# mehta-lab/dynamorph

Measured on AMD Instinct MI355X. Metric: cell-patches/sec (128x128x2) VQ-VAE fwd+bwd, higher is better.
Workload: dtype f32; 1 GPU; C3: VQ_VAE training step (forward + backward + fused Adam), 2x128x128 fp32 synthetic patches; per_gpu_batch=2048, global_batch=2048, parallelism=dp1, hip_graph=True, fused_trainer=True, backward_products=f32

## Files before the change

### dynamorph_amd/csrc/conv_mfma.hip

```cpp
#include "dm_common.h"
#include "tile.h"
#include "mfma_util.h"

int dm_generic_conv_slabs(int B, int per_tile);
int dm_generic_conv(int form, const Operand &in, const WeightView &wv, float *out, const Epilogue &ep, int B, int Cphys,
                    int CIN, int NOUT, int H, int W, int taps, int nslabs, int per_tile, hipStream_t st);
bool dm_wide_conv_ok(int form, int H, int W);
int dm_wide_conv_slabs(int form, int B, int H, int W, int per_tile);
long long dm_wide_conv_scratch_floats(int form, int CIN, int NOUT, int taps);
int dm_wide_conv(int form, const Operand &in, const WeightView &wv, float *scratch, float *out, const Epilogue &ep, int B,
                 int Cphys, int CIN, int NOUT, int H, int W, int taps, int nslabs, int per_tile, hipStream_t st);

bool dm_conv4x4s2_patch_forward(const Operand &in, const WeightView &wv, float *out, const Epilogue &ep, int B, int Cphys, int CIN,
                                int NOUT, int H, int W, int per_tile, int nslabs, hipStream_t stream, int *rc);

namespace {

enum { SIDE_NONE = 0, SIDE_MASK = 1, SIDE_ALL = 2 };

template <int SIDE> struct EpiIn { f32x4 m; };
template <> struct EpiIn<SIDE_ALL> { f32x4 m, r, q; };

constexpr unsigned DM_RSRC_FLAGS = 0x00020000u;
constexpr int DM_VOFF_NONE = 0x40000000;
// ... 533 lines not shown
        }
    }
    if (ep.stats && !(NPASS == 1 && per_tile)) {
        stats_reduce<NTT, PIX>(s1, s2, s_stat, ep, CO, blockIdx.x);
        zero_unowned_slabs(ep, CO, nslabs);
    }
}

template <int CIN, int COUT, int TH, int TW, bool TWO, int SIDE, int WPS>
__global__ __launch_bounds__(DM_BLOCK, WPS)
void convT_phase_kernel(Operand in, WeightView wv, float *__restrict__ out, Epilogue ep, int Cphys, int H, int W,
                        int ntiles, int nslabs)
{
    static_assert(COUT == 8 || COUT == 16, "built for 8 or 16 output channels");
    constexpr int IH = TH + 2, RS = TW + 8, COLS4 = RS / 4;
    constexpr int PSRAW = IH * RS;
    constexpr int PS = PSRAW + ((16 - (PSRAW % 32)) + 32) % 32;
    constexpr int CG = TW / 16, MT = TH * CG, MTW = MT / 4, MP = 2;
    constexpr int NPX = COUT == 16 ? 2 : 1;
    constexpr int TAPX = COUT == 16 ? 2 : 3;
    constexpr int KS = (CIN / 4) * 2 * TAPX;
    static_assert(CIN % 4 == 0 && MTW % MP == 0 && MTW >= MP, "shape");
    __shared__ __attribute__((aligned(16))) float tile[CIN * PS];
    __shared__ __attribute__((aligned(16))) float s_coef[DM_COEF_MAX_C * 4];
    __shared__ double s_stat[4 * 16][2];

    const int tiles_x = W / TW, tiles_y = H / TH;
    const int lane = threadIdx.x & 63, wave = threadIdx.x >> 6, m = lane & 15, kq = lane >> 4;
    const int OH = 2 * H, OW = 2 * W;
    const int co = COUT == 16 ? m : (m & 7), pxl = COUT == 16 ? 0 : (m >> 3);

    TileStage<CIN, IH, COLS4, RS, PS, TWO> stage;
    stage.init(H, W);
    int tidx = blockIdx.x, b = 0, y0 = 0, x0 = 0;
    if (tidx < ntiles) {
        int t = tidx;
        x0 = (t % tiles_x) * TW; t /= tiles_x;
        y0 = (t % tiles_y) * TH; b = t / tiles_y;
        stage.issue(in, b, Cphys, H, W, y0 - 1, x0 - 4);
        stage_coef(s_coef, in, b, Cphys);
    }

    float wreg[2][NPX][1][KS];
#pragma unroll
    for (int py = 0; py < 2; ++py)
#pragma unroll
        for (int pxt = 0; pxt < NPX; ++pxt)
#pragma unroll
            for (int s = 0; s < KS; ++s) {
                const int cg4 = s / (2 * TAPX), j = s % (2 * TAPX), a = j / TAPX, bb = j % TAPX;
                const int c = 4 * cg4 + kq;
                const int px = COUT == 16 ? pxt : pxl;
                const int row = py + a, col = COUT == 16 ? pxt + bb : bb;
                const int ky = py + 3 - 2 * row, kx = px + 3 - 2 * col;
                float wvl = 0.f;
                if (ky >= 0 && ky <= 3 && kx >= 0 && kx <= 3) wvl = wv.w[wv.off + co * wv.sn + c * wv.sc + ky * wv.sky + kx * wv.skx];
                wreg[py][pxt][0][s] = wvl;
            }
    const float bias = ep.bias ? ep.bias[co] : 0.f;
    float mc0, mc2;
    mask_coef(ep, 0, co, mc0, mc2);

    double s1 = 0.0, s2 = 0.0;
    const int abase = kq * PS + m + 3;
    EpiCtx<SIDE> cx;
    const long long sample_elems = (long long)COUT * OH * OW;
    const int chan_off = (co * OH * OW + 8 * kq + 4 * pxl) * 4;

    while (tidx < ntiles) {
        __syncthreads();
        stage.commit(tile, s_coef, Cphys, H, W, y0 - 1, x0 - 4, in.mode);
        __syncthreads();
        const int cb = b, cy0 = y0, cx0 = x0;
        const int next = tidx + gridDim.x;
        {
            int t = next < ntiles ? next : tidx;
            x0 = (t % tiles_x) * TW; t /= tiles_x;
            y0 = (t % tiles_y) * TH; b = t / tiles_y;
        }
        const auto scx = stage.begin(in, next < ntiles, b, Cphys, H, W, y0 - 1, x0 - 4);
        const bool recoef = next < ntiles && coef_changes(in, cb, b);
        f32x4 cfn = {1.f, 0.f, 0.f, 0.f};
        if (recoef) cfn = coef_fetch(in, b, Cphys);
        if (SIDE != SIDE_NONE && ep.mask.p0 && ep.mask.coef_bstride) mask_coef(ep, cb, co, mc0, mc2);
        cx.rebase(ep, out, sample_elems, cb);
        constexpr int NP = MTW / MP, NE = decltype(stage)::N;
#pragma unroll
        for (int p = 0; p < NP; ++p) {
#pragma unroll
            for (int e = 0; e < NE; ++e)
                if (e >= p * NE / NP && e < (p + 1) * NE / NP) stage.issue_one(e, scx);
            const float *ap[MP];
            int obase[MP];
#pragma unroll
            for (int i = 0; i < MP; ++i) {
                const int ti = wave + 4 * (MP * p + i);
                const int r = ti / CG, cg = ti % CG;
                ap[i] = tile + r * RS + 16 * cg + abase;
                obase[i] = chan_off + (2 * (cy0 + r) * OW + 2 * (cx0 + 16 * cg)) * 4;
            }
#pragma unroll
            for (int py = 0; py < 2; ++py) {
                EpiIn<SIDE> e[MP][NPX];
#pragma unroll
                for (int i = 0; i < MP; ++i)
#pragma unroll
                    for (int h = 0; h < NPX; ++h) epilogue_loads<SIDE>(e[i][h], cx, obase[i] + py * OW * 4 + 16 * h);
                f32x4 acc[NPX][MP][1];
#pragma unroll
                for (int pxt = 0; pxt < NPX; ++pxt) {
#pragma unroll
                    for (int i = 0; i < MP; ++i) acc[pxt][i][0] = (f32x4){0.f, 0.f, 0.f, 0.f};
                    auto off = [py, pxt](int s) {
                        const int cg4 = s / (2 * TAPX), j = s % (2 * TAPX), a = j / TAPX, bb = j % TAPX;
                        return 4 * cg4 * PS + (py + a) * RS + (COUT == 16 ? pxt + bb : bb);
                    };
                    mfma_tiles<MP, 1, KS, TAPX * 2>(ap, wreg[py][pxt], acc[pxt], off);
                }
#pragma unroll
                for (int i = 0; i < MP; ++i) {
                    if constexpr (COUT == 16) {
                        const f32x4 v0 = bias_relu(acc[0][i][0], ep, bias), v1 = bias_relu(acc[1][i][0], ep, bias);
                        epilogue_tail<SIDE>((f32x4){v0.x, v1.x, v0.y, v1.y}, ep, cx, e[i][0], mc0, mc2,
                                            obase[i] + py * OW * 4, s1, s2);
                        epilogue_tail<SIDE>((f32x4){v0.z, v1.z, v0.w, v1.w}, ep, cx, e[i][1], mc0, mc2,
                                            obase[i] + py * OW * 4 + 16, s1, s2);
                    } else {
                        const f32x4 v = bias_relu(acc[0][i][0], ep, bias);
                        const f32x4 pv = lane_xor8(v);
                        epilogue_tail<SIDE>(pxl ? (f32x4){pv.z, v.z, pv.w, v.w} : (f32x4){v.x, pv.x, v.y, pv.y}, ep, cx,
                                            e[i][0], mc0, mc2, obase[i] + py * OW * 4, s1, s2);
                    }
                }
            }
        }
        if (recoef) coef_put(s_coef, in, cfn, Cphys);
        tidx = next;
    }
    if (ep.stats) {
        double a = s1, c = s2;
        a += __shfl_xor(a, 16, 64); c += __shfl_xor(c, 16, 64);
        a += __shfl_xor(a, 32, 64); c += __shfl_xor(c, 32, 64);
        if (COUT == 8) { a += __shfl_xor(a, 8, 64); c += __shfl_xor(c, 8, 64); }
        if (lane < COUT) { s_stat[wave * 16 + lane][0] = a; s_stat[wave * 16 + lane][1] = c; }
        __syncthreads();
        if (threadIdx.x < COUT) {
            double ta = 0.0, tc = 0.0;
#pragma unroll
            for (int w = 0; w < 4; ++w) { ta += s_stat[w * 16 + threadIdx.x][0]; tc += s_stat[w * 16 + threadIdx.x][1]; }
            ep.stats[((long long)blockIdx.x * COUT + threadIdx.x) * 2 + 0] = ta;
            ep.stats[((long long)blockIdx.x * COUT + threadIdx.x) * 2 + 1] = tc;
        }
        zero_unowned_slabs(ep, COUT, nslabs);
    }
}

template <int CD, int CX, int TH, int TW>
struct FusedBwdGeom {
    static_assert(CD == 16 && CX == 8 && (TH == 8 || TH == 4) && TW % 16 == 0, "built for enc.4: 8 -> 16 channels");
    static constexpr int IH = TH + 2, RS = TW + 8, COLS4 = RS / 4, PSRAW = IH * RS;
    static constexpr int PS = PSRAW + ((16 - (PSRAW % 32)) + 32) % 32;
    static constexpr int TROWS = 2 * TH + 2, RST = 2 * TW + 8, TCOLS4 = RST / 4, PST = TROWS * RST;
    static constexpr int N = CX * 16, NTT = N / 16;
    static constexpr int TILE_FLOATS = CD * PS + CX * PST, RED_FLOATS = NTT * 256;
    static constexpr size_t LDS_BYTES = (size_t)(2 * TILE_FLOATS + 2 * DM_COEF_MAX_C * 4) * 4 + 8 * 16 * 2 * sizeof(double);
    static_assert(RED_FLOATS <= TILE_FLOATS, "the slab combine reuses a tile buffer");
};

template <int CD, int CX, int TH, int TW, bool ZF, bool DESC>
__global__ __launch_bounds__(768, 1)
void bwd_s2_roles3_kernel(Operand dy, Operand tin, WeightView wv, float *__restrict__ dx, Epilogue ep,
                         float *__restrict__ wslabs, int H, int W, int ntiles, int dbg)
{
    using G = FusedBwdGeom<CD, CX, TH, TW>;
    constexpr int RW = 4;
    constexpr int IH = G::IH, RS = G::RS, COLS4 = G::COLS4, PS = G::PS;
    constexpr int TROWS = G::TROWS, RST = G::RST, TCOLS4 = G::TCOLS4, PST = G::PST, NTT = G::NTT, N = G::N;
    constexpr int BUF = CD * PS + CX * PST;
    constexpr int CGN = TW / 16, MP = ZF ? CGN : 2, NPASS = TH * CGN / (RW * MP), WROWS = TH / RW;
    static_assert(TH * CGN == RW * MP * NPASS && TH == RW * WROWS, "tile split over the waves of a role");
    constexpr int TAPX = 3, KS = (CD / 4) * 2 * TAPX;
    extern __shared__ __attribute__((aligned(16))) float fb_lds[];
    float *s_coefD = fb_lds + 2 * BUF, *s_coefT = s_coefD + DM_COEF_MAX_C * 4;
    double (*s_stat)[2] = reinterpret_cast<double (*)[2]>(s_coefT + DM_COEF_MAX_C * 4);

    const int lane = threadIdx.x & 63, m = lane & 15, kq = lane >> 4;
    const int wave = __builtin_amdgcn_readfirstlane(threadIdx.x >> 6);
    const int role = wave / RW;
    const int rw = wave & (RW - 1);
    const int OH = 2 * H, OW = 2 * W;
    const int tiles_x = W / TW, tiles_y = H / TH;
    auto coords = [&](int kth, int &tb, int &ty0, int &tx0) {
        int t = tile_id<DESC>(kth, ntiles);
        tx0 = (t % tiles_x) * TW; t /= tiles_x;
        ty0 = (t % tiles_y) * TH; tb = t / tiles_y;
    };
    stage_coef(s_coefD, dy, 0, CD);
    stage_coef(s_coefT, tin, 0, CX);
    int tidx = blockIdx.x;

    if (role == 1) {
        TileStage<CD, IH, COLS4, RS, PS, true, 256> stD;
        TileStage<CX, TROWS, TCOLS4, RST, PST, false, 256> stT;
        const int tl = (int)threadIdx.x - 256;
        stD.init(H, W, tl);
        stT.init(OH, OW, tl);
        int b, y0, x0;
        if (tidx < ntiles) {
            coords(tidx, b, y0, x0);
            stD.issue(dy, b, CD, H, W, y0 - 1, x0 - 4);
        }
        __syncthreads();
        if (tidx < ntiles) {
            stD.commit(fb_lds, s_coefD, CD, H, W, y0 - 1, x0 - 4, dy.mode);
            stT.issue(tin, b, CX, OH, OW, 2 * y0 - 1, 2 * x0 - 4);
            stT.commit(fb_lds + CD * PS, s_coefT, CX, OH, OW, 2 * y0 - 1, 2 * x0 - 4, tin.mode);
        }
        __syncthreads();
        int p = 0;
        while (tidx < ntiles) {
            const int next = tidx + gridDim.x;
            float *nxt = fb_lds + (1 - p) * BUF;
            int nb = 0, ny0 = 0, nx0 = 0;
            if (next < ntiles && !(dbg & 4)) {
                coords(next, nb, ny0, nx0);
                stD.issue(dy, nb, CD, H, W, ny0 - 1, nx0 - 4);
                stD.commit(nxt, s_coefD, CD, H, W, ny0 - 1, nx0 - 4, dy.mode);
                stT.issue(tin, nb, CX, OH, OW, 2 * ny0 - 1, 2 * nx0 - 4);
                stT.commit(nxt + CD * PS, s_coefT, CX, OH, OW, 2 * ny0 - 1, 2 * nx0 - 4, tin.mode);
            }
            __syncthreads();
            p ^= 1;
            tidx = next;
        }
        for (int w = 0; w < RW + 2; ++w) __syncthreads();
    } else if (role == 2) {
        int bl[NTT];
#pragma unroll
        for (int t = 0; t < NTT; ++t) {
            const int n = 16 * t + m;
            bl[t] = CD * PS + (n >> 4) * PST + ((n >> 2) & 3) * RST + (n & 3) + 3 + 8 * kq + 2 * rw * RST;
        }
        const int al = m * PS + (rw + 1) * RS + 4 + 4 * kq;
        f32x4 wacc[NTT];
#pragma unroll
        for (int t = 0; t < NTT; ++t) wacc[t] = (f32x4){0.f, 0.f, 0.f, 0.f};
        __syncthreads();
        __syncthreads();
        int p = 0;
        while (tidx < ntiles) {
            const float *cur = fb_lds + p * BUF;
            if (!(dbg & 1)) {
                constexpr int NSPAN = TW / 16, NQ = WROWS * NSPAN * 4;
                auto aoff = [](int q) { return (q / (NSPAN * 4)) * RW * RS + 16 * ((q >> 2) % NSPAN); };
                auto boff = [](int q) { return (q / (NSPAN * 4)) * RW * 2 * RST + 32 * ((q >> 2) % NSPAN) + 2 * (q & 3); };
                f32x4 av[2];
                float bv[2][NTT];
                av[0] = *reinterpret_cast<const f32x4 *>(cur + al);
#pragma unroll
                for (int t = 0; t < NTT; ++t) bv[0][t] = cur[bl[t]];
#pragma unroll
                for (int q = 0; q < NQ; ++q) {
                    if (q + 1 < NQ) {
                        if (((q + 1) & 3) == 0) av[((q + 1) >> 2) & 1] = *reinterpret_cast<const f32x4 *>(cur + al + aoff(q + 1));
#pragma unroll
                        for (int t = 0; t < NTT; ++t) bv[(q + 1) & 1][t] = cur[bl[t] + boff(q + 1)];
                    }
                    __builtin_amdgcn_sched_barrier(0);
                    const float a = av[(q >> 2) & 1][q & 3];
#pragma unroll
                    for (int t = 0; t < NTT; ++t) wacc[t] = __builtin_amdgcn_mfma_f32_16x16x4f32(a, bv[q & 1][t], wacc[t], 0, 0, 0);
                    __builtin_amdgcn_sched_barrier(0);
                }
            }
            __syncthreads();
            p ^= 1;
            tidx += gridDim.x;
        }
        float *red = fb_lds;
        for (int w = 0; w < RW; ++w) {
            __syncthreads();
            if (rw == w) {
#pragma unroll
                for (int t = 0; t < NTT; ++t) {
                    f32x4 *pp = reinterpret_cast<f32x4 *>(red + (t * 64 + lane) * 4);
                    if (w == 0) *pp = wacc[t];
                    else *pp = *pp + wacc[t];
                }
            }
        }
        __syncthreads();
        __syncthreads();
    } else {
        const int co = m & 7, pxl = m >> 3;
        constexpr int NTW = ZF ? 2 : 1, KSW = ZF ? (CD / 4) * 2 : KS;
        float wreg[2][NTW][KSW];
#pragma unroll
        for (int py = 0; py < 2; ++py)
#pragma unroll
            for (int t = 0; t < NTW; ++t)
#pragma unroll
                for (int s = 0; s < KSW; ++s) {
                    int cg4, a, kx;
                    if constexpr (ZF) { cg4 = s >> 1; a = s & 1; kx = t == 0 ? 1 + pxl : (pxl ? 0 : 3); }
                    else { cg4 = s / (2 * TAPX); const int j = s % (2 * TAPX); a = j / TAPX; kx = pxl + 3 - 2 * (j % TAPX); }
                    const int c = 4 * cg4 + kq;
// ... 82 lines not shown
            p ^= 1;
            tidx += gridDim.x;
        }
        for (int w = 0; w < RW + 1; ++w) __syncthreads();
        if (ep.stats) {
            double a = s1, c = s2;
            a += __shfl_xor(a, 16, 64); c += __shfl_xor(c, 16, 64);
            a += __shfl_xor(a, 32, 64); c += __shfl_xor(c, 32, 64);
            a += __shfl_xor(a, 8, 64); c += __shfl_xor(c, 8, 64);
            if (lane < CX) { s_stat[rw * 16 + lane][0] = a; s_stat[rw * 16 + lane][1] = c; }
        }
        __syncthreads();
        if (ep.stats && threadIdx.x < CX) {
            double ta = 0.0, tc = 0.0;
#pragma unroll
            for (int w = 0; w < RW; ++w) { ta += s_stat[w * 16 + threadIdx.x][0]; tc += s_stat[w * 16 + threadIdx.x][1]; }
            ep.stats[((long long)blockIdx.x * CX + threadIdx.x) * 2 + 0] = ta;
            ep.stats[((long long)blockIdx.x * CX + threadIdx.x) * 2 + 1] = tc;
        }
    }
    float *slab = wslabs + (long long)blockIdx.x * (CD * N);
    for (int i = threadIdx.x; i < NTT * 256; i += 768) {
        const int j = i & 3, l = (i >> 2) & 63, t = i >> 8;
        slab[(4 * (l >> 4) + j) * N + 16 * t + (l & 15)] = fb_lds[i];
    }
}

struct ConvArgs {
    Operand in; WeightView wv; float *out; Epilogue ep;
    int B, Cphys, CIN, NOUT, H, W, per_tile;
    int ntiles, nslabs;
    hipStream_t stream;
};

int side_mode(const Epilogue &ep)
{
    if (!ep.mask.p0 && !ep.resid && !ep.stat_q) return SIDE_NONE;
    if (ep.mask.p0 && !ep.resid && (!ep.stat_q || ep.stat_q == ep.mask.p0)) return SIDE_MASK;
    return SIDE_ALL;
}

int conv_grid(int ntiles, int wgs_per_cu, int per_tile, int npass = 1)
{
    if (per_tile && npass > 1) return ntiles;
    const int cap = 256 * wgs_per_cu;
    return ntiles < cap ? ntiles : cap;
}

int conv_slabs(int ntiles, int per_tile) { return per_tile ? ntiles : (ntiles < 256 * 3 ? ntiles : 256 * 3); }

constexpr int lds_wgs(int lds_bytes) { return (160 * 1024) / (lds_bytes + 3072); }
constexpr int clampi(int v, int lo, int hi) { return v < lo ? lo : (v > hi ? hi : v); }

constexpr int conv_wps(int lds_bytes, int weights, int tile_f4, bool two, int mp, int nt, int side)
{
    const int stage = ((tile_f4 + DM_BLOCK - 1) / DM_BLOCK) * (two ? 9 : 5);
    const int epi = mp * nt * (6 + (side == SIDE_ALL ? 12 : (side == SIDE_MASK ? 4 : 0)));
    const int est = weights + stage + epi + 48;
    return clampi(lds_wgs(lds_bytes), 1, est > 145 ? 2 : 3);
}

int conv4_tw(int CIN, int Wo)
{
    const int cap = CIN <= 5 ? 64 : (CIN <= 8 ? 32 : 16);
    return Wo < cap ? Wo : cap;
}

constexpr bool CONV4_DESC = true;
constexpr bool FUSED_BWD_DESC = true;

template <int CIN, int TW>
void launch_conv4(const ConvArgs &a)
{
    constexpr int TH = 8;
    constexpr int F4 = CIN * (2 * TH + 2) * ((2 * TW + 8) / 4), LDS = 16 * F4;
#define DM_L4(SIDE_)                                                                                              \
    {                                                                                                             \
        constexpr int WPS = conv_wps(LDS, CIN * 4, F4, false, 2, 1, SIDE_);                                       \
                                            \
        if (SIDE_ == SIDE_NONE && CIN <= 4 && TW == 64 && a.NOUT == 8 && a.ep.bias_border && !a.ep.relu)          \
            hipLaunchKernelGGL((conv4x4s2_pair_kernel<CIN <= 4 ? CIN : 1, TH, WPS>),                              \
                               dim3(conv_grid(a.ntiles, WPS, a.per_tile)), dim3(DM_BLOCK), 0, a.stream, a.in, a.wv, \
                               a.out, a.ep, a.Cphys, a.H, a.W, a.ntiles, a.nslabs, a.per_tile);                   \
        else if (SIDE_ == SIDE_NONE && CIN <= 5 && a.ep.bias_border)                                              \
            hipLaunchKernelGGL((conv4x4s2_kernel<CIN, 1, TH, TW, SIDE_NONE, WPS, true, CONV4_DESC>),              \
                               dim3(conv_grid(a.ntiles, WPS, a.per_tile)), dim3(DM_BLOCK), 0, a.stream, a.in, a.wv, \
                               a.out, a.ep, a.Cphys, a.NOUT, a.H, a.W, a.ntiles, a.nslabs,                        \
                               a.per_tile);                                                                       \
        else                                                                                                      \
            hipLaunchKernelGGL((conv4x4s2_kernel<CIN, 1, TH, TW, SIDE_, WPS, false, CONV4_DESC>),                 \
                               dim3(conv_grid(a.ntiles, WPS, a.per_tile)), dim3(DM_BLOCK), 0, a.stream, a.in, a.wv, \
                               a.out, a.ep, a.Cphys, a.NOUT, a.H, a.W, a.ntiles, a.nslabs,                        \
                               a.per_tile);                                                                       \
    }
    switch (side_mode(a.ep)) {
    case SIDE_NONE: DM_L4(SIDE_NONE) break;
    case SIDE_MASK: DM_L4(SIDE_MASK) break;
    default: DM_L4(SIDE_ALL)
    }
#undef DM_L4
}

int conv3_tw(int W, int CIN)
{
    const int cap = CIN >= 32 ? 16 : (CIN >= 16 ? 32 : 64);
    return W < cap ? W : cap;
}
constexpr int conv3_th(int TW, int CIN) { return (TW == 16 && CIN < 32) ? 16 : 8; }

template <int CIN, int NT, int NPASS, int TAPS, bool PIX, int TW>
void launch_conv3(const ConvArgs &a)
{
    constexpr int TH = conv3_th(TW, CIN);
    constexpr int PADR = TAPS == 9 ? 1 : 0;
    constexpr int F4 = CIN * (TH + 2 * PADR) * ((TW + 8 * PADR) / 4), LDS = 16 * F4 + 2048;
    const int side = side_mode(a.ep);
    const bool two = a.in.mode == DM_LOAD_AFFINE2;
#define DM_L3(TWO_, SIDE_)                                                                                        \
    {                                                                                                             \
        constexpr int WPS = conv_wps(LDS, NT * (CIN / 4) * TAPS, F4, TWO_, NT == 1 ? 2 : 1, NT, SIDE_);           \
        hipLaunchKernelGGL((conv3x3_kernel<CIN, NT, NPASS, TAPS, PIX, TH, TW, TWO_, SIDE_, WPS>),                 \
                           dim3(conv_grid(a.ntiles, WPS, a.per_tile, NPASS)), dim3(DM_BLOCK), 0, a.stream, a.in, a.wv, \
                           a.out, a.ep, a.Cphys, a.NOUT, a.H, a.W, a.ntiles, a.nslabs, a.per_tile);               \
    }
    if (!two && side == SIDE_NONE) DM_L3(false, SIDE_NONE)
    else if (!two && side == SIDE_MASK) DM_L3(false, SIDE_MASK)
    else if (two && side != SIDE_ALL) DM_L3(true, SIDE_MASK)
    else DM_L3(true, SIDE_ALL)
#undef DM_L3
}

template <int CIN, int COUT, int TW>
void launch_convT_phase(const ConvArgs &a)
{
    constexpr int TH = conv3_th(TW, CIN);
    constexpr int F4 = CIN * (TH + 2) * ((TW + 8) / 4), LDS = 16 * F4 + 2048;
    constexpr int KSW = (CIN / 4) * (COUT == 16 ? 4 : 6) * (COUT == 16 ? 4 : 2);
    const int side = side_mode(a.ep);
    const bool two = a.in.mode == DM_LOAD_AFFINE2;
#define DM_LP(TWO_, SIDE_)                                                                                        \
    {                                                                                                             \
        constexpr int WPS = clampi(conv_wps(LDS, KSW, F4, TWO_, 2, COUT == 16 ? 2 : 1, SIDE_), 1, 2);             \
        hipLaunchKernelGGL((convT_phase_kernel<CIN, COUT, TH, TW, TWO_, SIDE_, WPS>),                             \
                           dim3(conv_grid(a.ntiles, WPS, a.per_tile)), dim3(DM_BLOCK), 0, a.stream, a.in, a.wv,   \
                           a.out, a.ep, a.Cphys, a.H, a.W, a.ntiles, a.nslabs);                                   \
    }
    if (!two && side == SIDE_NONE) DM_LP(false, SIDE_NONE)
    else if (!two && side == SIDE_MASK) DM_LP(false, SIDE_MASK)
    else if (two && side != SIDE_ALL) DM_LP(true, SIDE_MASK)
    else DM_LP(true, SIDE_ALL)
#undef DM_LP
}

}

static int conv_common_checks(const char *who, const dm_operand *in, const dm_weight_view *w, float *out,
                              const dm_epilogue *ep, int B, int CIN, int NOUT, int H, int W)
{
    if (dm_check_operand(in, who)) return -1;
    DM_REQUIRE(w && w->w && out, "%s: NULL weight or output", who);
    DM_REQUIRE(B > 0 && CIN > 0 && NOUT > 0 && H > 0 && W > 0, "%s: bad shape", who);
    DM_REQUIRE((long long)B * (CIN > NOUT ? CIN : NOUT) * H * W < (1LL << 31),
               "%s: tensor too large for 32-bit element offsets", who);
    DM_REQUIRE(CIN - (in->ones_channel ? 1 : 0) > 0, "%s: no physical input channel", who);
    DM_REQUIRE((long long)NOUT * H * W * 4 < DM_VOFF_NONE, "%s: one output sample must stay below 1 GiB", who);
    if (ep && ep->mask.p0 && dm_check_operand(&ep->mask, who)) return -1;
    DM_REQUIRE(!(ep && ep->mask.p0 && ep->mask.ones_channel), "%s: mask operand cannot have a ones channel", who);
    DM_REQUIRE(!(ep && ep->mask.p0 && ep->mask.mode != DM_LOAD_IDENT && ep->mask.mode != DM_LOAD_AFFINE),
               "%s: mask operand must be IDENT or AFFINE", who);
    return 0;
}

enum { ROUTE_RESIDENT, ROUTE_WIDE, ROUTE_GENERIC };
struct ConvRoute {
    int kind;
    int TW, TH, ntiles;
    int nslabs;
    bool wide_ok;
    long long wide_floats;
};

static ConvRoute conv_route(int form, int taps, bool resident, int TW, int TH, int B, int CIN, int NOUT, int H, int W, int per_tile)
{
    ConvRoute r{};
    r.wide_ok = dm_wide_conv_ok(form, H, W);
    r.wide_floats = r.wide_ok && CIN > 0 && NOUT > 0 ? dm_wide_conv_scratch_floats(form, CIN, NOUT, taps) : 0;
    r.kind = resident ? ROUTE_RESIDENT : (r.wide_ok ? ROUTE_WIDE : ROUTE_GENERIC);
    if (resident) {
        r.TW = TW; r.TH = TH;
        r.ntiles = B * ((form == 0 ? H / 2 : H) / TH) * ((form == 0 ? W / 2 : W) / TW);
    }
    r.nslabs = resident ? conv_slabs(r.ntiles, per_tile)
                        : (r.wide_ok ? dm_wide_conv_slabs(form, B, H, W, per_tile) : dm_generic_conv_slabs(B, per_tile));
    return r;
}

#define DM_CONV4_ROWS(X)                                                                   \
    X(3, 64) X(3, 32) X(3, 16)                                                             \
    X(4, 64) X(4, 32) X(4, 16)                                                             \
    X(5, 64) X(5, 32) X(5, 16)                                                             \
    X(2, 64) X(2, 32) X(2, 16)                                                             \
    X(1, 64) X(1, 32) X(1, 16)                                                             \
    X(8, 32) X(8, 16)                                                                      \
    X(16, 16)

static bool conv4_has_kernel(int CIN, int TW)
{
#define DM_C4(C, T) if (CIN == C && TW == T) return true;
    DM_CONV4_ROWS(DM_C4)
#undef DM_C4
    return false;
}

static void conv4_launch_resident(const ConvArgs &a, int TW)
{
#define DM_C4(C, T) if (a.CIN == C && TW == T) return launch_conv4<C, T>(a);
    DM_CONV4_ROWS(DM_C4)
#undef DM_C4
}

static ConvRoute conv4_route(int B, int CIN, int NOUT, int H, int W, int per_tile)
{
    const int Wo = W / 2, Ho = H / 2, TW = conv4_tw(CIN, Wo);
    const bool tileable = !(H % 16 || W % 32 || NOUT > 16 || (TW != 16 && TW != 32 && TW != 64) || Ho % 8 || Wo % TW);
    return conv_route(0, 16, tileable && conv4_has_kernel(CIN, TW), TW, 8, B, CIN, NOUT, H, W, per_tile);
}

static bool conv4_resident_takes(const dm_operand *in, const dm_epilogue *ep, int CIN, int W)
{
    const bool border_ok = !(ep && ep->bias_border) || (CIN <= 5 && !ep->mask.p0 && !ep->resid && !ep->stat_q && W / 2 >= 8);
    return in->mode != DM_LOAD_AFFINE2 && border_ok;
}

extern "C" int dm_conv4x4s2_num_blocks(int B, int CIN, int NOUT, int H, int W, int per_tile)
{
    if (B <= 0 || H <= 0 || W <= 0 || (H & 1) || (W & 1)) return -1;
    return conv4_route(B, CIN, NOUT, H, W, per_tile).nslabs;
}

extern "C" int64_t dm_conv4x4s2_scratch_floats(int CIN, int NOUT, int H, int W, int fallback)
{
    const ConvRoute r = conv4_route(1, CIN, NOUT, H, W, 0);
    return r.kind == ROUTE_RESIDENT && !fallback ? 0 : r.wide_floats;
}

extern "C" int dm_conv4x4s2(const dm_operand *in, const dm_weight_view *w, float *out, const dm_epilogue *ep,
                            int B, int CIN, int NOUT, int H, int W, void *stream)
{
    if (conv_common_checks("dm_conv4x4s2", in, w, out, ep, B, CIN, NOUT, H, W)) return -1;
    DM_REQUIRE(H % 2 == 0 && W % 2 == 0, "dm_conv4x4s2: H and W must be even (got %dx%d)", H, W);
    const int per_tile = ep ? ep->stats_per_tile : 0;
    const ConvRoute r = conv4_route(B, CIN, NOUT, H, W, per_tile);
    ConvArgs a{to_dev(in), to_dev(w), out, to_dev(ep), B, CIN - (in->ones_channel ? 1 : 0), CIN, NOUT, H, W,
               per_tile, r.ntiles, r.nslabs, (hipStream_t)stream};
    {
        int rc = 0;
        if (dm_conv4x4s2_patch_forward(a.in, a.wv, out, a.ep, B, a.Cphys, CIN, NOUT, H, W, per_tile, r.nslabs, a.stream, &rc))
            return rc;
    }
    if (r.kind == ROUTE_RESIDENT && conv4_resident_takes(in, ep, CIN, W))
        conv4_launch_resident(a, r.TW);
    else if (r.wide_ok && w->scratch && w->scratch_floats >= r.wide_floats)
        dm_wide_conv(0, a.in, a.wv, w->scratch, out, a.ep, B, a.Cphys, CIN, NOUT, H, W, 16, r.nslabs, per_tile, a.stream);
    else
        dm_generic_conv(0, a.in, a.wv, out, a.ep, B, a.Cphys, CIN, NOUT, H, W, 16, r.nslabs, per_tile, a.stream);
    return dm_launch_status("dm_conv4x4s2");
}

#define DM_CONVT_PHASE_ROWS(X) X(8, 16) X(8, 32) X(16, 16) X(16, 32)
#define DM_CONV3_ROWS(X)                                                                   \
                             \
    X(16, 1, 1, 1, 9, false, 16) X(16, 1, 1, 1, 9, false, 32)                              \
    X(16, 2, 2, 1, 9, false, 16) X(16, 2, 2, 1, 9, false, 32)                              \
    X(32, 1, 1, 1, 9, false, 16) X(32, 1, 1, 1, 9, false, 32)                              \
                                              \
    X(32, 1, 1, 1, 1, false, 16) X(32, 1, 1, 1, 1, false, 32)                              \
    X(16, 2, 2, 1, 1, false, 16) X(16, 2, 2, 1, 1, false, 32)                              \
     \
    X(16, 2, 2, 1, 9, true, 16) X(16, 2, 2, 1, 9, true, 32) X(16, 2, 2, 1, 9, true, 64)    \
    X(16, 4, 2, 2, 9, true, 16) X(16, 4, 2, 2, 9, true, 32)                                \
    X(8, 1, 1, 1, 9, true, 32) X(8, 1, 1, 1, 9, true, 64)                                  \
    X(4, 1, 1, 1, 9, true, 64)
#define DM_CP_IS(CO, T) (pix && CIN == 16 && NOUT == 4 * CO && TW == T && !per_tile)
#define DM_C3_IS(C, NTOT, TP, PX, T) (CIN == C && (NOUT + 15) / 16 == NTOT && taps == TP && pix == PX && TW == T)

static bool conv3_has_kernel(int CIN, int NOUT, int taps, bool pix, int per_tile, int TW)
{
#define DM_CP(CO, T) if (DM_CP_IS(CO, T)) return true;
#define DM_C3(C, NTOT, NT_, NP_, TP, PX, T) if (DM_C3_IS(C, NTOT, TP, PX, T)) return true;
    DM_CONVT_PHASE_ROWS(DM_CP)
    DM_CONV3_ROWS(DM_C3)
#undef DM_CP
#undef DM_C3
    return false;
}

static void conv3_launch_resident(const ConvArgs &a, int taps, bool pix, int TW)
{
    const int CIN = a.CIN, NOUT = a.NOUT, per_tile = a.per_tile;
#define DM_CP(CO, T) if (DM_CP_IS(CO, T)) return launch_convT_phase<16, CO, T>(a);
#define DM_C3(C, NTOT, NT_, NP_, TP, PX, T) if (DM_C3_IS(C, NTOT, TP, PX, T)) return launch_conv3<C, NT_, NP_, TP, PX, T>(a);
    DM_CONVT_PHASE_ROWS(DM_CP)
    DM_CONV3_ROWS(DM_C3)
#undef DM_CP
#undef DM_C3
}
#undef DM_CP_IS
#undef DM_C3_IS

static ConvRoute conv3_route(int B, int CIN, int NOUT, int H, int W, int taps, bool pix, int per_tile)
{
    const int TW = conv3_tw(W, CIN), TH = conv3_th(TW, CIN);
    const bool tileable = (TW == 16 || TW == 32 || TW == 64) && W % TW == 0 && H % TH == 0 && CIN % 4 == 0 && CIN <= 32;
    return conv_route(pix ? 2 : 1, taps, tileable && conv3_has_kernel(CIN, NOUT, taps, pix, per_tile, TW), TW, TH, B, CIN, NOUT,
                      H, W, per_tile);
}

extern "C" int dm_conv3x3_num_blocks(int B, int CIN, int NOUT, int H, int W, int taps, int pixel_shuffle, int per_tile)
{
    if (B <= 0 || H <= 0 || W <= 0) return -1;
    return conv3_route(B, CIN, NOUT, H, W, taps, pixel_shuffle != 0, per_tile).nslabs;
}

extern "C" int64_t dm_conv3x3_scratch_floats(int CIN, int NOUT, int H, int W, int taps, int pixel_shuffle, int per_tile)
{
    const ConvRoute r = conv3_route(1, CIN, NOUT, H, W, taps, pixel_shuffle != 0, per_tile);
    return r.kind == ROUTE_RESIDENT || (taps != 9 && taps != 1) ? 0 : r.wide_floats;
}

extern "C" int dm_conv3x3(const dm_operand *in, const dm_weight_view *w, float *out, const dm_epilogue *ep,
                          int B, int CIN, int NOUT, int H, int W, int taps, int pixel_shuffle, void *stream)
{
    if (conv_common_checks("dm_conv3x3", in, w, out, ep, B, CIN, NOUT, H, W)) return -1;
    DM_REQUIRE(taps == 9 || taps == 1, "dm_conv3x3: taps must be 9 or 1");
    DM_REQUIRE(!pixel_shuffle || (taps == 9 && NOUT % 4 == 0), "dm_conv3x3: pixel_shuffle needs taps=9, NOUT%%4==0");
    DM_REQUIRE(!in->ones_channel, "dm_conv3x3: ones_channel not supported");
    DM_REQUIRE(!(ep && ep->bias_border), "dm_conv3x3: bias_border not supported (dm_conv4x4s2 only)");
    const bool pix = pixel_shuffle != 0;
    const int form = pix ? 2 : 1, per_tile = ep ? ep->stats_per_tile : 0;
    const ConvRoute r = conv3_route(B, CIN, NOUT, H, W, taps, pix, per_tile);
    ConvArgs a{to_dev(in), to_dev(w), out, to_dev(ep), B, CIN, CIN, NOUT, H, W, per_tile, r.ntiles, r.nslabs,
               (hipStream_t)stream};
    if (r.kind == ROUTE_RESIDENT)
        conv3_launch_resident(a, taps, pix, r.TW);
    else if (r.wide_ok && w->scratch && w->scratch_floats >= r.wide_floats)
        dm_wide_conv(form, a.in, a.wv, w->scratch, out, a.ep, B, CIN, CIN, NOUT, H, W, taps, r.nslabs, per_tile, a.stream);
    else
        dm_generic_conv(form, a.in, a.wv, out, a.ep, B, CIN, CIN, NOUT, H, W, taps, r.nslabs, per_tile, a.stream);
    return dm_launch_status("dm_conv3x3");
}


static bool fused_bwd_shape(int CD, int CX, int H, int W)
{
    return CD == 16 && CX == 8 && H > 0 && W > 0 && H % 8 == 0 && W % 32 == 0;
}

extern "C" int dm_conv_bwd_s2_fused_supported(int CD, int CX, int H, int W) { return fused_bwd_shape(CD, CX, H, W) ? 1 : 0; }

extern "C" int dm_backward_precision(int mode)
{
    DM_REQUIRE(mode != 1, "dm_backward_precision: the split-bf16 gradient kernels are not built (retired: slower than the "
                          "exact fp32 path on these layer widths)");
    return 0;
}

extern "C" int dm_conv_bwd_s2_fused_num_blocks(int B, int CD, int CX, int H, int W)
{
    if (B <= 0 || !fused_bwd_shape(CD, CX, H, W)) return -1;
    const long long ntiles = (long long)B * (H / 8) * (W / 32);
    const long long cap = 256;
    return (int)(ntiles < cap ? ntiles : cap);
}

extern "C" int dm_conv_bwd_s2_fused(const dm_operand *dy, const dm_operand *tin, const dm_weight_view *w, float *dx,
                                    const dm_epilogue *ep, float *w_slabs, int B, int CD, int CX, int H, int W,
                                    void *stream)
{
    if (dm_check_operand(dy, "dm_conv_bwd_s2_fused(dy)") || dm_check_operand(tin, "dm_conv_bwd_s2_fused(in)")) return -1;
    DM_REQUIRE(w && w->w && dx && w_slabs && ep, "dm_conv_bwd_s2_fused: NULL pointer");
    DM_REQUIRE(fused_bwd_shape(CD, CX, H, W), "dm_conv_bwd_s2_fused: shape %d -> %d channels on %dx%d not built", CX, CD, H, W);
    DM_REQUIRE(B > 0 && (long long)B * CD * 4 * H * W < (1LL << 31), "dm_conv_bwd_s2_fused: tensor too large for 32-bit offsets");
    DM_REQUIRE(!dy->ones_channel && !tin->ones_channel && tin->mode != DM_LOAD_AFFINE2,
               "dm_conv_bwd_s2_fused: operand modes");
    DM_REQUIRE(dy->coef_bstride == 0 && tin->coef_bstride == 0, "dm_conv_bwd_s2_fused: batch-statistics coefficients only");
    DM_REQUIRE(ep->mask.p0 == tin->p0 && (!ep->stat_q || ep->stat_q == tin->p0) && !ep->resid && !ep->bias && !ep->relu &&
                   ep->mask.coef_bstride == 0,
               "dm_conv_bwd_s2_fused: the epilogue must mask by (and take its statistics against) the layer input");
    if (dm_check_operand(&ep->mask, "dm_conv_bwd_s2_fused(mask)")) return -1;
    using G = FusedBwdGeom<16, 8, 8, 32>;
    using G64 = FusedBwdGeom<16, 8, 4, 64>;
    constexpr auto kd32 = bwd_s2_roles3_kernel<16, 8, 8, 32, false, FUSED_BWD_DESC>;
    constexpr auto kd32z = bwd_s2_roles3_kernel<16, 8, 8, 32, true, FUSED_BWD_DESC>;
    constexpr auto kd64z = bwd_s2_roles3_kernel<16, 8, 4, 64, true, FUSED_BWD_DESC>;
    static DmPerDeviceOnce attr_set;
    if (attr_set.need()) {
        hipError_t e = hipFuncSetAttribute((const void *)kd32, hipFuncAttributeMaxDynamicSharedMemorySize, (int)G::LDS_BYTES);
        if (e == hipSuccess)
            e = hipFuncSetAttribute((const void *)kd32z, hipFuncAttributeMaxDynamicSharedMemorySize, (int)G::LDS_BYTES);
        if (e == hipSuccess)
            e = hipFuncSetAttribute((const void *)kd64z, hipFuncAttributeMaxDynamicSharedMemorySize, (int)G64::LDS_BYTES);
        if (e != hipSuccess) { dm_set_error("dm_conv_bwd_s2_fused: cannot reserve %zu bytes of LDS: %s", G::LDS_BYTES, hipGetErrorString(e)); return (int)e; }
        attr_set.mark();
    }
    const int ntiles = B * (H / 8) * (W / 32);
    const int grid = dm_conv_bwd_s2_fused_num_blocks(B, CD, CX, H, W);
    if (W == 64 && H % 4 == 0)
        hipLaunchKernelGGL(kd64z, dim3(grid), dim3(768), G64::LDS_BYTES, (hipStream_t)stream,
                           to_dev(dy), to_dev(tin), to_dev(w), dx, to_dev(ep), w_slabs, H, W, B * (H / 4), 0);
    else if (W == 32)
        hipLaunchKernelGGL(kd32z, dim3(grid), dim3(768), G::LDS_BYTES, (hipStream_t)stream,
                           to_dev(dy), to_dev(tin), to_dev(w), dx, to_dev(ep), w_slabs, H, W, ntiles, 0);
    else
        hipLaunchKernelGGL(kd32, dim3(grid), dim3(768), G::LDS_BYTES, (hipStream_t)stream,
                           to_dev(dy), to_dev(tin), to_dev(w), dx, to_dev(ep), w_slabs, H, W, ntiles, 0);
    return dm_launch_status("dm_conv_bwd_s2_fused");
}
```

Before: 1.106 million patches/s.

## Add shift-based MFMA kernels for stride-2 transposed conv in decoder

Adds specialized transposed-convolution kernels for 4 and 8 output channels. Each computes only the kernel taps that contribute to each output phase, and exchanges horizontal neighbor contributions across lanes with ds_bpermute instead of going through a full 3x3 pixel-shuffle conv. Dispatch routes matching decoder shapes (pixel-shuffle, no side inputs, no stats, full-width tiles) to the new kernels ahead of the existing phase and conv3 paths. The aim is to cut redundant MFMA work and LDS traffic in the upsampling layers. It adds complex lane-exchange and boundary handling that could be wrong at tile or row edges.

```diff
diff --git a/dynamorph_amd/csrc/conv_mfma.hip b/dynamorph_amd/csrc/conv_mfma.hip
--- a/dynamorph_amd/csrc/conv_mfma.hip
+++ b/dynamorph_amd/csrc/conv_mfma.hip
@@ -709,6 +709,292 @@
             ep.stats[((long long)blockIdx.x * COUT + threadIdx.x) * 2 + 1] = tc;
         }
         zero_unowned_slabs(ep, COUT, nslabs);
+    }
+}
+
+template <int CG>
+__device__ __forceinline__ void side_send(const f32x4 (&V)[CG], bool px, int nb_addr, float (&xs)[CG])
+{
+#pragma unroll
+    for (int i = 0; i < CG; ++i) {
+        float first = V[i].x;
+        asm("" : "+v"(first));
+        xs[i] = __builtin_bit_cast(float, __builtin_amdgcn_ds_bpermute(nb_addr, __builtin_bit_cast(int, px ? first : V[i].w)));
+    }
+}
+template <int CG>
+__device__ __forceinline__ void side_join(const f32x4 (&U)[CG], const f32x4 (&V)[CG], const float (&xs)[CG], bool px, bool wrap,
+                                          f32x4 (&o)[CG])
+{
+#pragma unroll
+    for (int i = 0; i < CG; ++i) {
+        float far = px ? (i + 1 < CG ? xs[i + 1 < CG ? i + 1 : i] : 0.f) : (i > 0 ? xs[i > 0 ? i - 1 : i] : 0.f);
+        const f32x4 v = V[i];
+        float vx = v.x, vy = v.y;
+        asm("" : "+v"(vx), "+v"(vy), "+v"(far));
+        const float e = wrap ? far : xs[i];
+        o[i] = U[i] + (px ? (f32x4){v.y, v.z, v.w, e} : (f32x4){e, vx, vy, v.z});
+    }
+}
+
+template <int CIN, int TH, int TW, int WPS>
+__global__ __launch_bounds__(DM_BLOCK, WPS)
+void convT_shift4_kernel(Operand in, WeightView wv, float *__restrict__ out, Epilogue ep, int Cphys, int H, int W, int ntiles)
+{
+    constexpr int COUT = 4, IH = TH + 1, RS = TW, COLS4 = RS / 4;
+    constexpr int PSRAW = IH * RS;
+    constexpr int PS = PSRAW + ((16 - (PSRAW % 32)) + 32) % 32;
+    constexpr int CG = TW / 16, C4 = CIN / 4, RPW = TH / 4;
+    static_assert(CIN % 4 == 0 && TH % 4 == 0 && TW % 16 == 0, "shape");
+    __shared__ __attribute__((aligned(16))) float tile[CIN * PS];
+    __shared__ __attribute__((aligned(16))) float s_coef[DM_COEF_MAX_C * 4];
+
+    const int tiles_y = H / TH;
+    const int lane = threadIdx.x & 63, wave = __builtin_amdgcn_readfirstlane(threadIdx.x >> 6), m = lane & 15, kq = lane >> 4;
+    const int OH = 2 * H, OW = 2 * W;
+    const int co = m >> 2;
+    const bool py = (m >> 1) & 1, px = m & 1;
+
+    TileStage<CIN, IH, COLS4, RS, PS, false> stage;
+    stage.init(H, W);
+    int tidx = blockIdx.x, b = 0, y0 = 0;
+    if (tidx < ntiles) {
+        y0 = (tidx % tiles_y) * TH; b = tidx / tiles_y;
+        stage.issue(in, b, Cphys, H, W, y0 - 1, 0);
+        stage_coef(s_coef, in, b, Cphys);
+    }
+
+    float wU[C4][2], wV[C4][2];
+#pragma unroll
+    for (int c4 = 0; c4 < C4; ++c4)
+#pragma unroll
+        for (int a = 0; a < 2; ++a) {
+            const int ky = a ? (py ? 2 : 3) : (py ? 0 : 1);
+            const long long base = wv.off + co * wv.sn + (4 * c4 + kq) * wv.sc + ky * wv.sky;
+            wU[c4][a] = wv.w[base + (px ? 2 : 1) * wv.skx];
+            wV[c4][a] = wv.w[base + (px ? 0 : 3) * wv.skx];
+        }
+    const float bias = ep.bias ? ep.bias[co] : 0.f;
+    const float *ap = tile + kq * PS + m + RPW * wave * RS;
+    const int nb_addr = ((px ? lane + 16 : lane - 16) & 63) * 4;
+    const bool wrap = px ? kq == 3 : kq == 0;
+    EpiCtx<SIDE_NONE> cx;
+    const long long sample_elems = (long long)COUT * OH * OW;
+    const int chan_off = ((co * OH - (py ? 1 : 0)) * OW + 8 * kq + 4 * (px ? 1 : 0)) * 4;
+
+    auto emit = [&](const f32x4 (&U)[CG], const f32x4 (&V)[CG], int k, bool valid) __attribute__((always_inline)) {
+        f32x4 o[CG];
+        float xs[CG];
+        side_send<CG>(V, px, nb_addr, xs);
+        side_join<CG>(U, V, xs, px, wrap, o);
+#pragma unroll
+        for (int i = 0; i < CG; ++i) {
+            const f32x4 v = bias_relu(o[i], ep, bias);
+            const f32x4 pv = lane_xor1(v);
+            const f32x4 q = px ? (f32x4){pv.z, v.z, pv.w, v.w} : (f32x4){v.x, pv.x, v.y, pv.y};
+            __builtin_amdgcn_raw_buffer_store_b128(q, cx.out_r, valid ? chan_off + (2 * k * OW + 32 * i) * 4 : DM_VOFF_NONE, 0, 0);
+        }
+    };
+
+    while (tidx < ntiles) {
+        __syncthreads();
+        stage.commit(tile, s_coef, Cphys, H, W, y0 - 1, 0, in.mode);
+        __syncthreads();
+        const int cb = b, cy0 = y0;
+        const int next = tidx + gridDim.x;
+        {
+            const int t = next < ntiles ? next : tidx;
+            y0 = (t % tiles_y) * TH; b = t / tiles_y;
+        }
+        const auto scx = stage.begin(in, next < ntiles, b, Cphys, H, W, y0 - 1, 0);
+        const bool recoef = next < ntiles && coef_changes(in, cb, b);
+        f32x4 cfn = {1.f, 0.f, 0.f, 0.f};
+        if (recoef) cfn = coef_fetch(in, b, Cphys);
+        cx.rebase(ep, out, sample_elems, cb);
+#pragma unroll
+        for (int e = 0; e < decltype(stage)::N; ++e) stage.issue_one(e, scx);
+        {
+            float av[RPW + 1][CG][C4];
+#pragma unroll
+            for (int r = 0; r <= RPW; ++r)
+#pragma unroll
+                for (int i = 0; i < CG; ++i)
+#pragma unroll
+                    for (int c4 = 0; c4 < C4; ++c4) av[r][i][c4] = ap[r * RS + 16 * i + 4 * c4 * PS];
+            constexpr int JB = CG <= 2 ? RPW : 1;
+#pragma unroll
+            for (int j0 = 0; j0 < RPW; j0 += JB) {
+                f32x4 U[JB][CG], V[JB][CG];
+#pragma unroll
+                for (int j = 0; j < JB; ++j)
+#pragma unroll
+                    for (int i = 0; i < CG; ++i) { U[j][i] = (f32x4){0.f, 0.f, 0.f, 0.f}; V[j][i] = (f32x4){0.f, 0.f, 0.f, 0.f}; }
+                __builtin_amdgcn_sched_barrier(0);
+#pragma unroll
+                for (int c4 = 0; c4 < C4; ++c4)
+#pragma unroll
+                    for (int a = 0; a < 2; ++a)
+#pragma unroll
+                        for (int j = 0; j < JB; ++j)
+#pragma unroll
+                            for (int i = 0; i < CG; ++i) {
+                                const float x = av[j0 + j + 1 - a][i][c4];
+                                U[j][i] = __builtin_amdgcn_mfma_f32_16x16x4f32(x, wU[c4][a], U[j][i], 0, 0, 0);
+                                V[j][i] = __builtin_amdgcn_mfma_f32_16x16x4f32(x, wV[c4][a], V[j][i], 0, 0, 0);
+                            }
+                __builtin_amdgcn_sched_barrier(0);
+#pragma unroll
+                for (int j = 0; j < JB; ++j) {
+                    const int k = cy0 + RPW * wave + j0 + j;
+                    emit(U[j], V[j], k, !(py && k == 0));
+                }
+            }
+        }
+        if (cy0 + TH == H && wave == (cb & 3)) {
+            f32x4 U[CG], V[CG];
+#pragma unroll
+            for (int i = 0; i < CG; ++i) { U[i] = (f32x4){0.f, 0.f, 0.f, 0.f}; V[i] = (f32x4){0.f, 0.f, 0.f, 0.f}; }
+            float av[CG][C4];
+#pragma unroll
+            for (int i = 0; i < CG; ++i)
+#pragma unroll
+                for (int c4 = 0; c4 < C4; ++c4) av[i][c4] = tile[kq * PS + m + TH * RS + 16 * i + 4 * c4 * PS];
+#pragma unroll
+            for (int c4 = 0; c4 < C4; ++c4)
+#pragma unroll
+                for (int i = 0; i < CG; ++i) {
+                    U[i] = __builtin_amdgcn_mfma_f32_16x16x4f32(av[i][c4], wU[c4][1], U[i], 0, 0, 0);
+                    V[i] = __builtin_amdgcn_mfma_f32_16x16x4f32(av[i][c4], wV[c4][1], V[i], 0, 0, 0);
+                }
+            emit(U, V, H, py);
+        }
+        if (recoef) coef_put(s_coef, in, cfn, Cphys);
+        tidx = next;
+    }
+}
+
+template <int CIN, int TH, int TW, int WPS>
+__global__ __launch_bounds__(DM_BLOCK, WPS)
+void convT_shift8_kernel(Operand in, WeightView wv, float *__restrict__ out, Epilogue ep, int Cphys, int H, int W, int ntiles)
+{
+    constexpr int COUT = 8, IH = TH + 2, RS = TW, COLS4 = RS / 4;
+    constexpr int PSRAW = IH * RS;
+    constexpr int PS = PSRAW + ((16 - (PSRAW % 32)) + 32) % 32;
+    constexpr int CG = TW / 16, C4 = CIN / 4, RPW = TH / 4;
+    static_assert(CIN % 4 == 0 && TH % 4 == 0 && TW % 16 == 0, "shape");
+    __shared__ __attribute__((aligned(16))) float tile[CIN * PS];
+    __shared__ __attribute__((aligned(16))) float s_coef[DM_COEF_MAX_C * 4];
+
+    const int tiles_y = H / TH;
+    const int lane = threadIdx.x & 63, wave = threadIdx.x >> 6, m = lane & 15, kq = lane >> 4;
+    const int OH = 2 * H, OW = 2 * W;
+    const int co = m & 7;
+    const bool px = m >> 3;
+
+    TileStage<CIN, IH, COLS4, RS, PS, false> stage;
+    stage.init(H, W);
+    int tidx = blockIdx.x, b = 0, y0 = 0;
+    if (tidx < ntiles) {
+        y0 = (tidx % tiles_y) * TH; b = tidx / tiles_y;
+        stage.issue(in, b, Cphys, H, W, y0 - 1, 0);
+        stage_coef(s_coef, in, b, Cphys);
+    }
+
+    float wU[2][C4][2], wV[2][C4][2];
+#pragma unroll
+    for (int py = 0; py < 2; ++py)
+#pragma unroll
+        for (int c4 = 0; c4 < C4; ++c4)
+#pragma unroll
+            for (int a = 0; a < 2; ++a) {
+                const int ky = a ? (py ? 0 : 3) : (py ? 2 : 1);
+                const long long base = wv.off + co * wv.sn + (4 * c4 + kq) * wv.sc + ky * wv.sky;
+                wU[py][c4][a] = wv.w[base + (px ? 2 : 1) * wv.skx];
+                wV[py][c4][a] = wv.w[base + (px ? 0 : 3) * wv.skx];
+            }
+    const float bias = ep.bias ? ep.bias[co] : 0.f;
+    const float *ap = tile + kq * PS + m + RPW * wave * RS;
+    const int nb_addr = ((px ? lane + 16 : lane - 16) & 63) * 4;
+    const bool wrap = px ? kq == 3 : kq == 0;
+    EpiCtx<SIDE_NONE> cx;
+    const long long sample_elems = (long long)COUT * OH * OW;
+    const int chan_off = (co * OH * OW + 8 * kq + 4 * (px ? 1 : 0)) * 4;
+
+    while (tidx < ntiles) {
+        __syncthreads();
+        stage.commit(tile, s_coef, Cphys, H, W, y0 - 1, 0, in.mode);
+        __syncthreads();
+        const int cb = b, cy0 = y0;
+        const int next = tidx + gridDim.x;
+        {
+            const int t = next < ntiles ? next : tidx;
+            y0 = (t % tiles_y) * TH; b = t / tiles_y;
+        }
+        const auto scx = stage.begin(in, next < ntiles, b, Cphys, H, W, y0 - 1, 0);
+        const bool recoef = next < ntiles && coef_changes(in, cb, b);
+        f32x4 cfn = {1.f, 0.f, 0.f, 0.f};
+        if (recoef) cfn = coef_fetch(in, b, Cphys);
+        cx.rebase(ep, out, sample_elems, cb);
+        float av[RPW + 2][CG][C4];
+#pragma unroll
+        for (int r = 0; r < RPW + 2; ++r)
+#pragma unroll
+            for (int i = 0; i < CG; ++i)
+#pragma unroll
+                for (int c4 = 0; c4 < C4; ++c4) av[r][i][c4] = ap[r * RS + 16 * i + 4 * c4 * PS];
+        constexpr int NE = decltype(stage)::N;
+        f32x4 U[2][2][CG], V[2][2][CG];
+#pragma unroll
+        for (int j = 0; j <= RPW; ++j) {
+            float xs[2][CG];
+            if (j > 0) {
+#pragma unroll
+                for (int py = 0; py < 2; ++py) side_send<CG>(V[(j - 1) & 1][py], px, nb_addr, xs[py]);
+            }
+            if (j < RPW) {
+#pragma unroll
+                for (int e = 0; e < NE; ++e)
+                    if (e >= j * NE / RPW && e < (j + 1) * NE / RPW) stage.issue_one(e, scx);
+#pragma unroll
+                for (int py = 0; py < 2; ++py)
+#pragma unroll
+                    for (int i = 0; i < CG; ++i) {
+                        U[j & 1][py][i] = (f32x4){0.f, 0.f, 0.f, 0.f};
+                        V[j & 1][py][i] = (f32x4){0.f, 0.f, 0.f, 0.f};
+                    }
+                __builtin_amdgcn_sched_barrier(0);
+#pragma unroll
+                for (int c4 = 0; c4 < C4; ++c4)
+#pragma unroll
+                    for (int a = 0; a < 2; ++a)
+#pragma unroll
+                        for (int py = 0; py < 2; ++py)
+#pragma unroll
+                            for (int i = 0; i < CG; ++i) {
+                                const float x = av[j + 1 + (a ? (py ? 1 : -1) : 0)][i][c4];
+                                U[j & 1][py][i] = __builtin_amdgcn_mfma_f32_16x16x4f32(x, wU[py][c4][a], U[j & 1][py][i], 0, 0, 0);
+                                V[j & 1][py][i] = __builtin_amdgcn_mfma_f32_16x16x4f32(x, wV[py][c4][a], V[j & 1][py][i], 0, 0, 0);
+                            }
+                __builtin_amdgcn_sched_barrier(0);
+            }
+            if (j > 0) {
+#pragma unroll
+                for (int py = 0; py < 2; ++py) {
+                    f32x4 o[CG];
+                    side_join<CG>(U[(j - 1) & 1][py], V[(j - 1) & 1][py], xs[py], px, wrap, o);
+#pragma unroll
+                    for (int i = 0; i < CG; ++i) {
+                        const f32x4 v = bias_relu(o[i], ep, bias);
+                        const f32x4 pv = lane_xor8(v);
+                        const f32x4 q = px ? (f32x4){pv.z, v.z, pv.w, v.w} : (f32x4){v.x, pv.x, v.y, pv.y};
+                        __builtin_amdgcn_raw_buffer_store_b128(
+                            q, cx.out_r, chan_off + ((2 * (cy0 + RPW * wave + j - 1) + py) * OW + 32 * i) * 4, 0, 0);
+                    }
+                }
+            }
+        }
+        if (recoef) coef_put(s_coef, in, cfn, Cphys);
+        tidx = next;
     }
 }
 
@@ -1097,6 +1383,18 @@
 #undef DM_LP
 }
 
+template <int CIN, int COUT, int TW>
+void launch_convT_shift(const ConvArgs &a)
+{
+    constexpr int TH = conv3_th(TW, CIN), WPS = COUT == 4 ? 3 : 2;
+    if constexpr (COUT == 4)
+        hipLaunchKernelGGL((convT_shift4_kernel<CIN, TH, TW, WPS>), dim3(conv_grid(a.ntiles, WPS, 0)), dim3(DM_BLOCK), 0, a.stream,
+                           a.in, a.wv, a.out, a.ep, a.Cphys, a.H, a.W, a.ntiles);
+    else
+        hipLaunchKernelGGL((convT_shift8_kernel<CIN, TH, TW, WPS>), dim3(conv_grid(a.ntiles, WPS, 0)), dim3(DM_BLOCK), 0, a.stream,
+                           a.in, a.wv, a.out, a.ep, a.Cphys, a.H, a.W, a.ntiles);
+}
+
 }
 
 static int conv_common_checks(const char *who, const dm_operand *in, const dm_weight_view *w, float *out,
@@ -1226,6 +1524,8 @@
     X(16, 4, 2, 2, 9, true, 16) X(16, 4, 2, 2, 9, true, 32)                                \
     X(8, 1, 1, 1, 9, true, 32) X(8, 1, 1, 1, 9, true, 64)                                  \
     X(4, 1, 1, 1, 9, true, 64)
+#define DM_CONVT_SHIFT_ROWS(X) X(8, 4, 32) X(16, 8, 16) X(8, 4, 64) X(16, 8, 32)
+#define DM_CS_IS(C, CO, T) (shift_ops && CIN == C && NOUT == 4 * CO && TW == T && a.W == T)
 #define DM_CP_IS(CO, T) (pix && CIN == 16 && NOUT == 4 * CO && TW == T && !per_tile)
 #define DM_C3_IS(C, NTOT, TP, PX, T) (CIN == C && (NOUT + 15) / 16 == NTOT && taps == TP && pix == PX && TW == T)
 
@@ -1243,6 +1543,10 @@
 static void conv3_launch_resident(const ConvArgs &a, int taps, bool pix, int TW)
 {
     const int CIN = a.CIN, NOUT = a.NOUT, per_tile = a.per_tile;
+    const bool shift_ops = pix && !per_tile && side_mode(a.ep) == SIDE_NONE && !a.ep.stats && a.in.mode != DM_LOAD_AFFINE2;
+#define DM_CS(C, CO, T) if (DM_CS_IS(C, CO, T)) return launch_convT_shift<C, CO, T>(a);
+    DM_CONVT_SHIFT_ROWS(DM_CS)
+#undef DM_CS
 #define DM_CP(CO, T) if (DM_CP_IS(CO, T)) return launch_convT_phase<16, CO, T>(a);
 #define DM_C3(C, NTOT, NT_, NP_, TP, PX, T) if (DM_C3_IS(C, NTOT, TP, PX, T)) return launch_conv3<C, NT_, NP_, TP, PX, T>(a);
     DM_CONVT_PHASE_ROWS(DM_CP)
@@ -1250,6 +1554,7 @@
 #undef DM_CP
 #undef DM_C3
 }
+#undef DM_CS_IS
 #undef DM_CP_IS
 #undef DM_C3_IS
 
```

Result: faster. 1.119 million patches/s, median of 6 (+1.1%).
